# FriedFeid/Video-Depth-Anything

Measured on AMD Instinct MI355X. Metric: depth frames/sec at 32x518x518, ViT-L fp16, 1/2/4/8 MI355X, higher is better.
Workload: dtype fp16; 1 GPU; VideoDepthAnything.forward vitl 1x32x3x518x518 per GPU; encoder=vitl, frames_per_clip=32, H=518, W=518, clips_per_gpu=1, parallelism=clip-parallel dp1, ranks=1, depth_gather_to_rank0=False, hip_graph=False, clips_in_flight=2

## Files before the change

include/vda_tune.h:

```cpp
#ifndef VDA_TUNE_H
#define VDA_TUNE_H
#include <stdint.h>
#ifdef __cplusplus
extern "C" {
#endif

int vda_debug_force_tile(int32_t cfg);
int vda_debug_gemm_sched(int32_t persist_blocks);
int vda_debug_strip_split(int32_t nsplit);
int vda_debug_hconv(int32_t mode);
int vda_debug_dconv(int32_t mode);
int vda_debug_attn(int32_t temporal_direct);

#ifdef __cplusplus
}
#endif
#endif
```

video-depth-anything_amd/_lib.py:

```python
from __future__ import annotations

import ctypes
import os
from ctypes import c_float, c_int32, c_int64, c_void_p, POINTER

_HERE = os.path.dirname(os.path.abspath(__file__))
LIB_PATH = os.environ.get("VDA_LIB_OVERRIDE") or os.path.join(_HERE, "libvda.so")
TORCH_LIB_PATH = os.path.join(_HERE, "libvda_torch.so")
if os.environ.get("VDA_LIB_OVERRIDE"):
    _ov = os.path.join(os.path.dirname(os.path.abspath(os.environ["VDA_LIB_OVERRIDE"])), "libvda_torch.so")
    if os.path.exists(_ov):
        TORCH_LIB_PATH = _ov

EXPORTED = (
    "vda_version", "vda_epilogue_size", "vda_last_error", "vda_gemm", "vda_gemm_check", "vda_conv2d", "vda_conv2d_workspace",
    "vda_layernorm",
    "vda_conv2d_res2_upsample_ok", "vda_conv2d_bias9_ok",
    "vda_subpixel_conv", "vda_subpixel_conv_workspace", "vda_subpixel_conv_check",
    "vda_row_stats", "vda_groupnorm", "vda_groupnorm_workspace",
    "vda_groupnorm_linear", "vda_groupnorm_linear_workspace", "vda_groupnorm_linear_fused",
    "vda_spatial_attention", "vda_temporal_attention", "vda_upsample_bilinear", "vda_patch_im2col",
    "vda_depth_head", "vda_depth_head_workspace", "vda_preprocess_frames", "vda_depth_resize",
    "vda_scale_shift", "vda_scale_shift_workspace", "vda_depth_align",
    "vda_depth_eval_workspace", "vda_depth_eval_fit", "vda_depth_eval_metrics",
    "vda_depth_range_workspace", "vda_depth_range", "vda_depth_colorize_bytes", "vda_depth_colorize",
    "vda_tile_size", "vda_depth_absdiff_range_workspace", "vda_depth_absdiff_range", "vda_panel_compose_bytes",
    "vda_panel_compose",
    "vda_yuv_to_rgb", "vda_preprocess_yuv_workspace", "vda_preprocess_yuv",
    "vda_resample_taps", "vda_resample_tables", "vda_yuv_downscale_ok", "vda_yuv_downscale_workspace",
    "vda_yuv_downscale",
    "vda_gemm_f32", "vda_conv2d_f32", "vda_layernorm_f32", "vda_groupnorm_f32", "vda_spatial_attention_f32",
    "vda_temporal_attention_f32", "vda_upsample_bilinear_f32", "vda_patch_im2col_f32", "vda_depth_head_f32",
)
TUNE_EXPORTED = ("vda_debug_force_tile", "vda_debug_gemm_sched", "vda_debug_strip_split", "vda_debug_hconv",
                 "vda_debug_dconv", "vda_debug_attn")
TUNE_LIB_PATH = os.path.join(os.path.dirname(_HERE), "build", "tune", "libvda.so")

ACT_NONE, ACT_GELU, ACT_GEGLU, ACT_RELU, ACT_SWIGLU = 0, 1, 2, 3, 4
STORE_ROWS, STORE_PIXEL_SHUFFLE = 0, 1
VIS_INDEX, VIS_HWC, VIS_PLANAR444, VIS_PLANAR420 = 0, 1, 2, 3
TILE_RGB, TILE_DEPTH, TILE_ERROR, TILE_XT = 0, 1, 2, 3
YUV_420, YUV_422, YUV_444, YUV_MONO = 0, 1, 2, 3


class VDAUnavailable(RuntimeError):
    pass


class VDAError(RuntimeError):
    pass


class Epilogue(ctypes.Structure):
    _fields_ = [
        ("bias", c_void_p), ("rowbias", c_void_p), ("rdiv", c_int32), ("rmod", c_int32),
        ("gamma", c_void_p), ("res", c_void_p), ("ldres", c_int64), ("res2", c_void_p),
        ("ldres2", c_int64), ("act", c_int32), ("store", c_int32), ("ps_k", c_int32),
        ("ps_cout", c_int32), ("ps_hin", c_int32), ("ps_win", c_int32),
        ("ln_stats", c_void_p), ("ln_colsum", c_void_p), ("ln_parts", c_int32), ("ln_eps", c_float),
        ("stats_out", c_void_p), ("res2_h", c_int32), ("res2_w", c_int32), ("sched", c_void_p),
        ("drop_period", c_int32), ("bias9", c_void_p),
    ]


class Tile(ctypes.Structure):
    _fields_ = [
        ("kind", c_int32), ("row", c_int32), ("col", c_int32), ("offset", c_int32), ("frames", c_int32),
        ("lut", c_int32), ("a", c_void_p), ("b", c_void_p), ("valid", c_void_p), ("range", c_void_p),
    ]


_lib = None
_load_error = None


def _declare(lib):
    P, I, L, F = c_void_p, c_int32, c_int64, c_float
    EP = POINTER(Epilogue)
    sig = {
        "vda_version": ([], ctypes.c_char_p),
        "vda_epilogue_size": ([], L),
        "vda_last_error": ([], ctypes.c_char_p),
        "vda_gemm": ([P, L, P, P, L, I, I, I, EP, P], I),
        "vda_gemm_check": ([L, L, I, I, I, EP], I),
        "vda_conv2d": ([P, P, P, I, I, I, I, I, I, I, I, I, I, I, EP, P, L, P], I),
        "vda_conv2d_workspace": ([I, I, I, I, I, I, I, I], L),
        "vda_conv2d_res2_upsample_ok": ([I, I, I, I, I, I, I, I], I),
        "vda_conv2d_bias9_ok": ([I, I, I, I, I, I, I], I),
        "vda_subpixel_conv": ([P, P, P, P, I, I, I, I, I, I, P, L, P], I),
        "vda_subpixel_conv_workspace": ([I, I, I, I, I], L),
        "vda_subpixel_conv_check": ([I, I, I, I, I, I], I),
        "vda_layernorm": ([P, L, P, P, P, I, I, F, I, P], I),
        "vda_row_stats": ([P, L, P, I, I, F, P], I),
        "vda_groupnorm": ([P, P, P, P, I, I, I, I, F, P, P], I),
        "vda_groupnorm_workspace": ([I, I, I, I], L),
        "vda_groupnorm_linear": ([P, P, P, I, I, I, I, F, P, P, P, I, P, P, L, P], I),
        "vda_groupnorm_linear_workspace": ([I, I, I, I, I], L),
        "vda_groupnorm_linear_fused": ([I, I, I], I),
        "vda_spatial_attention": ([P, P, I, I, I, I, F, P], I),
        "vda_temporal_attention": ([P, P, I, I, I, I, I, F, F, P], I),
        "vda_upsample_bilinear": ([P, P, I, I, I, I, I, I, P], I),
        "vda_patch_im2col": ([P, P, I, I, I, I, P], I),
        "vda_depth_head": ([P, P, P, P, P, P, P, I, I, I, I, I, I, P], I),
        "vda_depth_head_workspace": ([I, I, I, I, I, I], L),
        "vda_preprocess_frames": ([P, P, I, I, I, I, I, POINTER(F), POINTER(F), P], I),
        "vda_depth_resize": ([P, P, I, I, I, I, I, P], I),
        "vda_scale_shift_workspace": ([L], L),
        "vda_scale_shift": ([P, P, P, L, P, P, P, L, P], I),
        "vda_depth_align": ([P, I, I, I, I, I, P, I, P, POINTER(F), POINTER(F), P, P], I),
        "vda_depth_eval_workspace": ([I, L], L),
        "vda_depth_eval_fit": ([P, P, P, I, L, I, P, P, P, L, P], I),
        "vda_depth_eval_metrics": ([P, P, P, I, L, P, I, F, P, P, P, P, L, P], I),
        "vda_depth_range_workspace": ([L], L),
        "vda_depth_range": ([P, L, P, P, L, P], I),
        "vda_depth_colorize_bytes": ([I, I, I, I], L),
        "vda_depth_colorize": ([P, I, I, I, P, P, I, P, P], I),
        "vda_tile_size": ([], L),
        "vda_depth_absdiff_range_workspace": ([L], L),
        "vda_depth_absdiff_range": ([P, P, P, L, P, P, L, P], I),
        "vda_panel_compose_bytes": ([I, I, I, I, I, I], L),
        "vda_panel_compose": ([POINTER(Tile), I, I, I, I, I, I, I, I, I, P, P, I, P, P], I),
        "vda_yuv_to_rgb": ([P, I, I, I, L, I, P, P], I),
        "vda_preprocess_yuv_workspace": ([I, I, I, I, I], L),
        "vda_preprocess_yuv": ([P, I, I, I, L, I, P, I, I, POINTER(F), POINTER(F), P, L, P], I),
        "vda_resample_taps": ([I, I], I),
        "vda_resample_tables": ([I, I, P, P], I),
        "vda_yuv_downscale_ok": ([I, I, I, I], I),
        "vda_yuv_downscale_workspace": ([I, I, I, I, I], L),
        "vda_yuv_downscale": ([P, I, I, I, L, I, P, P, P, P, P, I, I, P, L, P], I),
        "vda_gemm_f32": ([P, L, P, P, L, I, I, I, EP, P], I),
        "vda_conv2d_f32": ([P, P, P, I, I, I, I, I, I, I, I, I, EP, P], I),
        "vda_layernorm_f32": ([P, L, P, P, P, I, I, F, I, P], I),
        "vda_groupnorm_f32": ([P, P, P, P, I, I, I, I, F, P], I),
        "vda_spatial_attention_f32": ([P, P, I, I, I, I, F, P], I),
        "vda_temporal_attention_f32": ([P, P, I, I, I, I, I, F, F, P], I),
        "vda_upsample_bilinear_f32": ([P, P, I, I, I, I, I, I, P], I),
        "vda_patch_im2col_f32": ([P, P, I, I, I, I, P], I),
        "vda_depth_head_f32": ([P, P, P, P, P, P, P, P, I, I, I, I, I, I, P], I),
        "vda_debug_force_tile": ([I], I),
        "vda_debug_gemm_sched": ([I], I),
        "vda_debug_strip_split": ([I], I),
        "vda_debug_hconv": ([I], I),
        "vda_debug_dconv": ([I], I),
        "vda_debug_attn": ([I], I),
    }
    for name, (args, res) in sig.items():
        if name.startswith("vda_debug_") and not hasattr(lib, name):
            continue
        fn = getattr(lib, name)
        fn.argtypes = args
        fn.restype = res


def lib():
    global _lib, _load_error
    if _lib is not None:
        return _lib
    if _load_error is not None:
        raise VDAUnavailable(_load_error)
    if not os.path.exists(LIB_PATH):
        _load_error = f"libvda.so not found at {LIB_PATH}; run `make` (or __graft_entry__.build())"
        raise VDAUnavailable(_load_error)
    try:
        l = ctypes.CDLL(LIB_PATH)
        _declare(l)
        if l.vda_epilogue_size() != ctypes.sizeof(Epilogue):
            raise OSError(f"vda_epilogue is {l.vda_epilogue_size()} bytes in the library, {ctypes.sizeof(Epilogue)} "
                          f"in _lib.Epilogue: rebuild libvda.so or update the mirror")
        if l.vda_tile_size() != ctypes.sizeof(Tile):
            raise OSError(f"vda_tile is {l.vda_tile_size()} bytes in the library, {ctypes.sizeof(Tile)} in _lib.Tile: "
                          f"rebuild libvda.so or update the mirror")
    except OSError as e:
        _load_error = f"failed to load {LIB_PATH}: {e}"
        raise VDAUnavailable(_load_error) from e
    _lib = l
    return _lib


_torch_ops = None


def torch_ops():
    global _torch_ops
    if _torch_ops is not None:
        return _torch_ops
    lib()
    if not os.path.exists(TORCH_LIB_PATH):
        raise VDAUnavailable(f"libvda_torch.so not found at {TORCH_LIB_PATH}; run `make` (or __graft_entry__.build())")
    import torch
    try:
        torch.ops.load_library(TORCH_LIB_PATH)
    except OSError as e:
        raise VDAUnavailable(f"failed to load {TORCH_LIB_PATH}: {e}") from e
    _torch_ops = torch.ops.vda
    return _torch_ops


def check(rc: int, what: str):
    if rc != 0:
        msg = lib().vda_last_error().decode(errors="replace")
        raise VDAError(f"{what} failed (rc={rc}): {msg}")
```

video-depth-anything_amd/csrc/vda_conv2d.hip:

```cpp
#include "vda_internal.h"

static bool conv_takes_strip(int BT, int H, int W, int Cin, int Cout, int ks, int stride, int pad, int up_h) {
  if (up_h > 0 || ks != 3 || stride != 1 || pad != 1 || !vda_conv_strip_serves(W, Cin, Cout)) return false;
  const long strip_tiles = (long)BT * ((H * W + 255) / 256);
  return g_force_tile == -3 || (g_force_tile == -1 && (Cin >= 512 || strip_tiles * 2 <= vda_cu_count()));
}

static long conv_im2col_bytes(int BT, int H, int W, int Cin, int ks, int stride, int pad) {
  const long Ho = (H + 2L * pad - ks) / stride + 1, Wo = (W + 2L * pad - ks) / stride + 1;
  return (long)BT * Ho * Wo * ks * ks * Cin * 2;
}
static bool conv_takes_im2col(int BT, int H, int W, int Cin, int Cout, int ks, int stride, int pad, int up_h) {
  if (up_h > 0 || ks != 3 || stride != 2 || Cout % 256 != 0 || g_force_tile != -1) return false;
  const long Ho = (H + 2L * pad - ks) / stride + 1, Wo = (W + 2L * pad - ks) / stride + 1;
  return Ho > 0 && Wo > 0 && vda_gemm_phased256_serves((long)BT * Ho * Wo, Cout, 9L * Cin, 9L * Cin);
}

static bool conv_takes_hconv(int BT, int H, int W, int Cin, int Cout, int ks, int stride, int pad) {
  return ks == 3 && stride == 1 && pad == 1 && g_force_tile == -1 && vda_conv_hconv_serves(BT, H, W, Cin, Cout);
}

extern "C" int64_t vda_conv2d_workspace(int32_t BT, int32_t H, int32_t W, int32_t Cin, int32_t Cout, int32_t ks,
                                        int32_t stride, int32_t pad) {
  if (BT <= 0 || H <= 0 || W <= 0 || Cin <= 0 || Cout <= 0) return 0;
  if (conv_takes_hconv(BT, H, W, Cin, Cout, ks, stride, pad)) return 0;
  if (conv_takes_im2col(BT, H, W, Cin, Cout, ks, stride, pad, 0)) return conv_im2col_bytes(BT, H, W, Cin, ks, stride, pad);
  if (!conv_takes_strip(BT, H, W, Cin, Cout, ks, stride, pad, 0)) return 0;
  return vda_conv_strip_ws_bytes(BT, H, W, Cin, Cout);
}

extern "C" int vda_conv2d_res2_upsample_ok(int32_t BT, int32_t H, int32_t W, int32_t Cin, int32_t Cout, int32_t ks,
                                           int32_t stride, int32_t pad) {
  if (BT <= 0 || H <= 0 || W <= 0 || Cin <= 0 || Cout <= 0) return 0;
  return conv_takes_hconv(BT, H, W, Cin, Cout, ks, stride, pad) ? 1 : 0;
}

extern "C" int vda_conv2d_bias9_ok(int32_t BT, int32_t H, int32_t W, int32_t Cin, int32_t Cout, int32_t up_h,
                                   int32_t up_w) {
  if (BT <= 0 || H <= 0 || W <= 0 || Cin <= 0 || Cout <= 0 || up_h <= 0 || up_w <= 0 || g_force_tile >= 0) return 0;
  return vda_conv_halo_fused_serves(BT, H, W, up_h, up_w, Cin, Cout) ? 1 : 0;
}

extern "C" int vda_conv2d(const void* x, const void* w, void* y, int32_t BT, int32_t H, int32_t W,
                          int32_t Cin, int32_t Cout, int32_t ks, int32_t stride, int32_t pad,
                          int32_t pre_relu, int32_t up_h, int32_t up_w, const vda_epilogue* epi,
                          void* ws, int64_t ws_bytes, void* stream) {
  VDA_CHECK_ARG(x && w && y, "null pointer");
  VDA_CHECK_ARG(BT > 0 && H > 0 && W > 0 && Cin > 0 && Cout > 0 && ks > 0 && stride > 0 && pad >= 0,
                "bad conv geometry");
  VDA_CHECK_ARG(Cin % 8 == 0 && Cout % 4 == 0, "Cin % 8 and Cout % 4 required");
  const int Hi = up_h > 0 ? up_h : H, Wi = up_w > 0 ? up_w : W;
  GemmParams p{};
  p.x = (const h16*)x; p.w = (const h16*)w; p.y = (h16*)y;
  p.H = H; p.W = W; p.Cin = Cin; p.ks = ks; p.stride = stride; p.pad = pad; p.pre_relu = pre_relu;
  p.up_h = up_h > 0 ? up_h : 0; p.up_w = up_w > 0 ? up_w : 0;
  p.Ho = (Hi + 2 * pad - ks) / stride + 1;
  p.Wo = (Wi + 2 * pad - ks) / stride + 1;
  VDA_CHECK_ARG(p.Ho > 0 && p.Wo > 0, "empty conv output");
  p.M = BT * p.Ho * p.Wo; p.N = Cout; p.K = ks * ks * Cin;
  p.ldy = Cout; p.ldx = 0;
  p.epi = epi ? *epi : vda_default_epi();
  if (p.epi.rdiv <= 0) p.epi.rdiv = 1;
  if (p.epi.rmod <= 0) p.epi.rmod = 1;
  VDA_CHECK_ARG(p.epi.store == VDA_STORE_ROWS && (p.epi.act == VDA_ACT_NONE || p.epi.act == VDA_ACT_RELU),
                "conv: row store, activation none/relu");
  VDA_CHECK_ARG(!p.epi.stats_out && !p.epi.ln_stats, "conv: no LayerNorm fold / row statistics");
  int rc = vda_check_epi(p.epi, p.M, Cout);
  if (rc) return rc;
  const bool res2_up = p.epi.res2_h > 0 || p.epi.res2_w > 0;
  if (res2_up) {
    VDA_CHECK_ARG(p.epi.res2 && p.epi.res2_h > 0 && p.epi.res2_w > 0 && p.epi.ldres2 == Cout && p.up_h == 0 &&
                      !p.epi.gamma && !p.epi.rowbias && (!p.epi.res || p.epi.ldres == Cout) &&
                      p.epi.res2_h <= p.Ho && p.epi.res2_w <= p.Wo &&
                      (long)p.epi.res2_h * p.epi.res2_w * Cout * 2 < (1L << 31) &&
                      conv_takes_hconv(BT, H, W, Cin, Cout, ks, stride, pad),
                  "upsampled res2 needs the halo conv route (vda_conv2d_res2_upsample_ok), a [BT, h <= Ho, w <= Wo, "
                  "Cout] source, no gamma / rowbias / input upsample");
    return vda_conv_hconv(x, w, y, p.epi.bias, p.epi.act == VDA_ACT_RELU, pre_relu, p.epi.res, p.epi.res2,
                          p.epi.res2_h, p.epi.res2_w, BT, H, W, Cin, Cout, (hipStream_t)stream);
  }
  VDA_CHECK_ARG(!p.epi.bias9 || (!p.epi.bias && (uintptr_t)p.epi.bias9 % 16 == 0 && ks == 3 && stride == 1 && pad == 1 &&
                                 !pre_relu && !p.epi.res && !p.epi.res2 && !p.epi.gamma && !p.epi.rowbias &&
                                 vda_conv2d_bias9_ok(BT, H, W, Cin, Cout, p.up_h, p.up_w)),
                "bias9: the 3x3 conv through a fused resize only (vda_conv2d_bias9_ok), 16-byte aligned, in place "
                "of bias, no residual / gamma / rowbias / pre-ReLU");
  if (p.up_h > 0) {
    if (g_force_tile < 0 && ks == 3 && stride == 1 && pad == 1 && !pre_relu && !p.epi.res && !p.epi.res2 &&
        !p.epi.gamma && !p.epi.rowbias) {
      rc = vda_conv_halo_fused(x, w, y, p.epi.bias, p.epi.act == VDA_ACT_RELU, BT, H, W, p.up_h, p.up_w, Cin, Cout,
                               (hipStream_t)stream, p.epi.bias9);
      if (rc != 1) return rc;
    }
    return vda_launch_conv_reg(p, (hipStream_t)stream);
  }
  if (!p.epi.gamma && !p.epi.rowbias && (!p.epi.res || p.epi.ldres == Cout) && (!p.epi.res2 || p.epi.ldres2 == Cout) &&
      conv_takes_hconv(BT, H, W, Cin, Cout, ks, stride, pad)) {
    rc = vda_conv_hconv(x, w, y, p.epi.bias, p.epi.act == VDA_ACT_RELU, pre_relu, p.epi.res, p.epi.res2, 0, 0, BT, H,
                        W, Cin, Cout, (hipStream_t)stream);
    if (rc != 1) return rc;
  }
  if (conv_takes_strip(BT, H, W, Cin, Cout, ks, stride, pad, 0) && !p.epi.gamma && !p.epi.rowbias &&
      (!p.epi.res || p.epi.ldres == Cout) && (!p.epi.res2 || p.epi.ldres2 == Cout)) {
    rc = vda_conv_strip(x, w, y, p.epi.bias, p.epi.act == VDA_ACT_RELU, pre_relu, p.epi.res, p.epi.res2, BT, H, W,
                        Cin, Cout, ws, ws ? ws_bytes : 0, (hipStream_t)stream);
    if (rc != 1) return rc;
  }
  if (g_force_tile < 0 && ks == 3 && stride == 1 && pad == 1 && !pre_relu && !p.epi.res && !p.epi.res2 &&
      !p.epi.gamma && !p.epi.rowbias && (long)H * W >= 128L * 128L) {
    rc = vda_conv_halo(x, w, y, p.epi.bias, p.epi.act == VDA_ACT_RELU, BT, H, W, Cin, Cout, (hipStream_t)stream);
    if (rc != 1) return rc;
  }
  if (conv_takes_im2col(BT, H, W, Cin, Cout, ks, stride, pad, 0) && !pre_relu && ws &&
      ws_bytes >= conv_im2col_bytes(BT, H, W, Cin, ks, stride, pad) && (uintptr_t)ws % 16 == 0 &&
      (uintptr_t)x % 16 == 0) {
    rc = vda_conv_im2col(x, ws, BT, H, W, Cin, p.Ho, p.Wo, ks, stride, pad, (hipStream_t)stream);
    if (rc) return rc;
    p.x = (const h16*)ws;
    p.ldx = p.K;
    return vda_launch_gemm(p, (hipStream_t)stream);
  }
  return vda_launch_conv_gemm(p, (hipStream_t)stream);
}
```

video-depth-anything_amd/csrc/vda_internal.h:

```cpp
#pragma once
#include "vda_common.h"
#include "../../include/vda.h"
static_assert(vda_glu(VDA_ACT_GEGLU) && vda_glu(VDA_ACT_SWIGLU) && !vda_glu(VDA_ACT_GELU) && !vda_glu(VDA_ACT_RELU),
              "vda_glu (vda_common.h) names the gated activation codes of vda.h");

struct GemmParams {
  const h16* x; long ldx;
  const h16* w;
  h16* y; long ldy;
  int M, N, K;
  int H, W, Cin, Ho, Wo, ks, stride, pad, pre_relu, up_h, up_w;
  vda_epilogue epi;
  int sp_bt, sp_phases;
  const float* sp_bias;
};
VDA_KNOB_DECL(int, g_force_tile, -1);
vda_epilogue vda_default_epi();
int vda_check_epi(const vda_epilogue& e, int M, int N);
int vda_launch_gemm(const GemmParams& p, hipStream_t st);
int vda_launch_conv_gemm(const GemmParams& p, hipStream_t st);
bool vda_gemm_phased256_serves(long M, long N, long K, long ldx);
int vda_launch_subpixel_gemm(const GemmParams& p, hipStream_t st);
int vda_launch_conv_reg(const GemmParams& p, hipStream_t st);
int vda_launch_depth_gemm(const GemmParams& p, hipStream_t st);

int vda_conv_halo(const void* x, const void* w, void* y, const float* bias, int relu, int BT, int H, int W, int Cin,
                  int Cout, hipStream_t st);
int vda_conv_halo_fused(const void* x, const void* w, void* y, const float* bias, int relu, int BT, int Hs, int Ws,
                        int H, int W, int Cin, int Cout, hipStream_t st, const float* bias9 = nullptr);
bool vda_conv_halo_fused_serves(int BT, int Hs, int Ws, int H, int W, int Cin, int Cout);

bool vda_depth_conv_serves(int H, int W, int C);
int vda_depth_conv(const void* U, const void* w1, const float* b1, const float* w2, const float* b2, float* depth,
                   int BT, int H, int W, int C, hipStream_t st);
bool vda_depth_conv_fused_serves(int Hs, int Ws, int H, int W, int C);
int vda_depth_conv_fused(const void* x, const void* w1, const float* b1, const float* w2, const float* b2,
                         float* depth, int BT, int Hs, int Ws, int H, int W, int C, hipStream_t st);

bool vda_conv_strip_serves(int W, int Cin, int Cout);
long vda_conv_strip_ws_bytes(int BT, int H, int W, int Cin, int Cout);
int vda_conv_strip(const void* x, const void* w, void* y, const float* bias, int relu_out, int pre_relu,
                   const void* res, const void* res2, int BT, int H, int W, int Cin, int Cout, void* ws,
                   long ws_bytes, hipStream_t st);

bool vda_conv_hconv_serves(int BT, int H, int W, int Cin, int Cout);
int vda_conv_hconv(const void* x, const void* w, void* y, const float* bias, int relu_out, int pre_relu,
                   const void* res, const void* res2, int res2_h, int res2_w, int BT, int H, int W, int Cin, int Cout,
                   hipStream_t st);

int vda_row_partials_launch(const void* y, int64_t ldy, float* out, int32_t rows, int32_t N, hipStream_t st);

int vda_conv_im2col(const void* x, void* a, int BT, int H, int W, int Cin, int Ho, int Wo, int ks, int stride, int pad,
                    hipStream_t st);
```

Baseline: 725.1 frames/s.

## Add source-resolution conv kernel for upsample-then-3x3-conv with Cout 128

Adds a kernel that evaluates a 3x3 conv on a 2x bilinearly upsampled input by running the GEMM on the low-resolution source tile, once per tap, and then applying the separable bilinear weights to the partial results. This cuts the MFMA work to roughly a quarter of convolving the upsampled image and avoids materialising the upsampled halo. The tap outputs are rounded to fp16 in LDS before interpolation, and the path is gated to exact 2x align-corners geometry with Cout=128, Cin<=256 and bias9 present by default. The kernel is tried ahead of the existing halo-fused path.

After: 735.0 frames/s, median of 6. 1.01x the previous value.

```diff
diff --git a/include/vda_tune.h b/include/vda_tune.h
--- a/include/vda_tune.h
+++ b/include/vda_tune.h
@@ -10,6 +10,7 @@
 int vda_debug_strip_split(int32_t nsplit);
 int vda_debug_hconv(int32_t mode);
 int vda_debug_dconv(int32_t mode);
+int vda_debug_oc1_src(int32_t mode);
 int vda_debug_attn(int32_t temporal_direct);
 
 #ifdef __cplusplus
diff --git a/video-depth-anything_amd/_lib.py b/video-depth-anything_amd/_lib.py
--- a/video-depth-anything_amd/_lib.py
+++ b/video-depth-anything_amd/_lib.py
@@ -33,7 +33,7 @@
     "vda_temporal_attention_f32", "vda_upsample_bilinear_f32", "vda_patch_im2col_f32", "vda_depth_head_f32",
 )
 TUNE_EXPORTED = ("vda_debug_force_tile", "vda_debug_gemm_sched", "vda_debug_strip_split", "vda_debug_hconv",
-                 "vda_debug_dconv", "vda_debug_attn")
+                 "vda_debug_dconv", "vda_debug_attn", "vda_debug_oc1_src")
 TUNE_LIB_PATH = os.path.join(os.path.dirname(_HERE), "build", "tune", "libvda.so")
 
 ACT_NONE, ACT_GELU, ACT_GEGLU, ACT_RELU, ACT_SWIGLU = 0, 1, 2, 3, 4
@@ -143,6 +143,7 @@
         "vda_debug_hconv": ([I], I),
         "vda_debug_dconv": ([I], I),
         "vda_debug_attn": ([I], I),
+        "vda_debug_oc1_src": ([I], I),
     }
     for name, (args, res) in sig.items():
         if name.startswith("vda_debug_") and not hasattr(lib, name):
diff --git a/video-depth-anything_amd/csrc/vda_conv2d.hip b/video-depth-anything_amd/csrc/vda_conv2d.hip
--- a/video-depth-anything_amd/csrc/vda_conv2d.hip
+++ b/video-depth-anything_amd/csrc/vda_conv2d.hip
@@ -87,6 +87,9 @@
   if (p.up_h > 0) {
     if (g_force_tile < 0 && ks == 3 && stride == 1 && pad == 1 && !pre_relu && !p.epi.res && !p.epi.res2 &&
         !p.epi.gamma && !p.epi.rowbias) {
+      rc = vda_conv_oc1_src(x, w, y, p.epi.bias, p.epi.act == VDA_ACT_RELU, BT, H, W, p.up_h, p.up_w, Cin, Cout,
+                            (hipStream_t)stream, p.epi.bias9);
+      if (rc != 1) return rc;
       rc = vda_conv_halo_fused(x, w, y, p.epi.bias, p.epi.act == VDA_ACT_RELU, BT, H, W, p.up_h, p.up_w, Cin, Cout,
                                (hipStream_t)stream, p.epi.bias9);
       if (rc != 1) return rc;
diff --git a/video-depth-anything_amd/csrc/vda_internal.h b/video-depth-anything_amd/csrc/vda_internal.h
--- a/video-depth-anything_amd/csrc/vda_internal.h
+++ b/video-depth-anything_amd/csrc/vda_internal.h
@@ -30,6 +30,10 @@
                         int H, int W, int Cin, int Cout, hipStream_t st, const float* bias9 = nullptr);
 bool vda_conv_halo_fused_serves(int BT, int Hs, int Ws, int H, int W, int Cin, int Cout);
 
+bool vda_conv_oc1_src_serves(int BT, int Hs, int Ws, int H, int W, int Cin, int Cout, bool bias9);
+int vda_conv_oc1_src(const void* x, const void* w, void* y, const float* bias, int relu, int BT, int Hs, int Ws, int H,
+                     int W, int Cin, int Cout, hipStream_t st, const float* bias9 = nullptr);
+
 bool vda_depth_conv_serves(int H, int W, int C);
 int vda_depth_conv(const void* U, const void* w1, const float* b1, const float* w2, const float* b2, float* depth,
                    int BT, int H, int W, int C, hipStream_t st);
diff --git a/video-depth-anything_amd/csrc/vda_oc1_src.hip b/video-depth-anything_amd/csrc/vda_oc1_src.hip
--- /dev/null
+++ b/video-depth-anything_amd/csrc/vda_oc1_src.hip
@@ -0,0 +1,348 @@
+#include <cmath>
+#include "vda_internal.h"
+#include "vda_halo.h"
+
+namespace {
+
+__device__ __attribute__((aligned(64))) uint4 g_sz_page[4];
+
+constexpr int ST = 16;
+constexpr int FP = 10;
+constexpr int FPIX = FP * FP;
+constexpr int MROWS = 128;
+constexpr int CMAX = 256;
+constexpr int CS = 64;
+constexpr int CO = 128;
+constexpr int CPX = CS / 8;
+constexpr int ZSTR = 132;
+constexpr int XBUF = MROWS * CMAX;
+constexpr int WBUF = CO * CS;
+constexpr int ZBUF = FPIX * ZSTR;
+constexpr int WPCS = CO * CPX / 64;
+constexpr int WPW = WPCS / 8;
+constexpr int SPS = 2;
+constexpr int WSLOT = SPS * WBUF;
+constexpr int WRING = 2;
+
+#ifndef VDA_OC1S_ABLATE
+#define VDA_OC1S_ABLATE 0
+#endif
+
+typedef unsigned u32x2 __attribute__((ext_vector_type(2)));
+
+__device__ __forceinline__ int w_pos(int n, int cd) { return cd ^ ((n >> 1) & (CPX - 1)); }
+
+__device__ __forceinline__ void slot_weights(int o, int out, int in, float sc, int g, float& a, float& b) {
+  int i0, i1;
+  float w;
+  ac_coord(min(max(o, 0), out - 1), in, sc, i0, i1, w);
+  const float u = 1.f - w;
+  const bool ok = (unsigned)o < (unsigned)out;
+  a = ok ? (i0 == g ? u : 0.f) + (i1 == g ? w : 0.f) : 0.f;
+  b = ok ? (i0 == g + 1 ? u : 0.f) + (i1 == g + 1 ? w : 0.f) : 0.f;
+}
+
+__global__ __launch_bounds__(512) void oc1_src_kernel(const h16* __restrict__ x, const h16* __restrict__ w1,
+                                                      const float* __restrict__ b1, const float* __restrict__ b9,
+                                                      h16* __restrict__ yout, int relu_out, int Hs, int Ws, int C,
+                                                      int tiles_x, int tiles_y, int ntiles) {
+  __shared__ __attribute__((aligned(16))) h16 xbuf[XBUF];
+  __shared__ __attribute__((aligned(16))) h16 wbuf[WRING * WSLOT];
+  __shared__ __attribute__((aligned(16))) h16 zbuf[ZBUF];
+  __shared__ float2 vtab[ST + 2];
+
+  const int tid = threadIdx.x, lane = tid & 63;
+  const int wave = __builtin_amdgcn_readfirstlane(tid >> 6);
+  const int ng = wave & 3, mh = wave >> 2;
+  const int frow = lane & 15, g = lane >> 4;
+  const int H = 2 * Hs, W = 2 * Ws;
+  const int nslab = C / CS;
+  const int K = 9 * C;
+  const int my_tiles = blockIdx.x < ntiles ? (ntiles - 1 - blockIdx.x) / gridDim.x + 1 : 0;
+  if (my_tiles == 0) return;
+  const void* zero = (const void*)g_sz_page;
+  const float usy = ac_scale(Hs, H), usx = ac_scale(Ws, W);
+
+  auto x_rows = [&](int bt, int y0, int x0, const h16* (&xp)[WPW]) {
+    const int by = y0 / 2 - 1, bx = x0 / 2 - 1;
+#pragma unroll
+    for (int j = 0; j < WPW; ++j) {
+      const int s = (wave * WPW + j) * 64 + lane;
+      const int row = s / CPX, cd = w_pos(row, s % CPX);
+      const int r = row / FP, c = row - r * FP;
+      const int gy = by + r, gx = bx + c;
+      const bool ok = row < FPIX && (unsigned)gy < (unsigned)Hs && (unsigned)gx < (unsigned)Ws;
+      xp[j] = ok ? x + (((long)bt * Hs + gy) * Ws + gx) * C + cd * 8 : nullptr;
+    }
+  };
+  auto dma_x_step = [&](const h16* const (&xp)[WPW], int st) {
+#pragma unroll
+    for (int sub = 0; sub < SPS; ++sub) {
+      const int slab = st * SPS + sub;
+#pragma unroll
+      for (int j = 0; j < WPW; ++j)
+        glds16(xp[j] && slab < nslab ? (const void*)(xp[j] + slab * CS) : zero,
+               xbuf + slab * WBUF + (wave * WPW + j) * 512);
+    }
+  };
+  const h16* wrow[WPW];
+#pragma unroll
+  for (int j = 0; j < WPW; ++j) {
+    const int s = (wave * WPW + j) * 64 + lane;
+    const int n = s / CPX, pos = s - n * CPX;
+    wrow[j] = w1 + (long)n * K + w_pos(n, pos) * 8;
+  }
+  const int nstep = (nslab + SPS - 1) / SPS;
+  int pf_tile = 0, pf_tap = 0, pf_step = 0, pf_slot = 0;
+  auto fetch_w = [&]() {
+    if (pf_tile >= my_tiles) return false;
+#if !(VDA_OC1S_ABLATE & 4)
+#pragma unroll
+    for (int sub = 0; sub < SPS; ++sub) {
+      const int slab = pf_step * SPS + sub;
+      const unsigned off = (unsigned)(pf_tap * C + slab * CS);
+#pragma unroll
+      for (int j = 0; j < WPW; ++j)
+        glds16(slab < nslab ? (const void*)(wrow[j] + off) : zero,
+               wbuf + pf_slot * WSLOT + sub * WBUF + (wave * WPW + j) * 512);
+    }
+#endif
+    if (++pf_step == nstep) {
+      pf_step = 0;
+      if (++pf_tap == 9) {
+        pf_tap = 0;
+        ++pf_tile;
+      }
+    }
+    if (++pf_slot == WRING) pf_slot = 0;
+    return true;
+  };
+
+  const int n0r = ng * 32 + frow;
+  unsigned lin_w[2];
+#pragma unroll
+  for (int d = 0; d < 2; ++d)
+    lin_w[d] = (unsigned)(uintptr_t)(VDA_LDS h16*)wbuf + (unsigned)(n0r * CPX + w_pos(n0r, d * 4 + g)) * 16u;
+  unsigned lin_x[2];
+#pragma unroll
+  for (int d = 0; d < 2; ++d)
+    lin_x[d] = (unsigned)(uintptr_t)(VDA_LDS h16*)xbuf +
+               (unsigned)((mh * 64 + frow) * CPX + w_pos(mh * 64 + frow, d * 4 + g)) * 16u;
+  const int xl = tid >> 5, cg = tid & 31;
+
+  const float* bsrc = b9 ? b9 + 4 * CO : b1;
+  const f4 bias_r = bsrc ? *reinterpret_cast<const f4*>(bsrc + cg * 4) : f4{0.f, 0.f, 0.f, 0.f};
+
+  float acc[ST][4];
+#pragma unroll
+  for (int i = 0; i < ST; ++i)
+#pragma unroll
+    for (int c = 0; c < 4; ++c) acc[i][c] = 0.f;
+
+  int bt, y0, x0;
+  halo_tile_of(blockIdx.x, tiles_x, tiles_y, ST, bt, y0, x0);
+  const h16* nxp[WPW];
+  x_rows(bt, y0, x0, nxp);
+  for (int st = 0; st < nstep; ++st) dma_x_step(nxp, st);
+#pragma unroll
+  for (int k = 0; k < WRING - 1; ++k) fetch_w();
+  wait_vmcnt<0>();
+  __builtin_amdgcn_s_barrier();
+
+  int rd_slot = 0;
+  for (int ti = 0; ti < my_tiles; ++ti) {
+    const bool more = ti + 1 < my_tiles;
+    int nbt = 0, ny0 = 0, nx0 = 0;
+    if (more) halo_tile_of(blockIdx.x + (ti + 1) * gridDim.x, tiles_x, tiles_y, ST, nbt, ny0, nx0);
+    if (tid < ST + 2) {
+      float a, b;
+      slot_weights(y0 - 1 + tid, H, Hs, usy, y0 / 2 - 1 + (tid >> 1), a, b);
+      vtab[tid] = make_float2(a, b);
+    }
+    float hA[3], hB[3];
+#pragma unroll
+    for (int tx = 0; tx < 3; ++tx)
+      slot_weights(x0 - 1 + xl + tx, W, Ws, usx, x0 / 2 - 1 + ((xl + tx) >> 1), hA[tx], hB[tx]);
+
+    float hs[FP][4];
+#pragma unroll
+    for (int tap = 0; tap < 9; ++tap) {
+      const int ty = tap / 3, tx = tap % 3;
+      f4 za[2][4];
+#pragma unroll
+      for (int a = 0; a < 2; ++a)
+#pragma unroll
+        for (int i = 0; i < 4; ++i) za[a][i] = f4{0.f, 0.f, 0.f, 0.f};
+      if (tap == 8 && more) x_rows(nbt, ny0, nx0, nxp);
+      for (int st = 0; st < nstep; ++st) {
+        fetch_w();
+        const bool xs = tap == 8 && more && st > 0;
+        if (xs) dma_x_step(nxp, st - 1);
+#if !(VDA_OC1S_ABLATE & 1)
+#pragma unroll
+        for (int d = 0; d < 2 * SPS; ++d) {
+          const int slab = st * SPS + (d >> 1);
+          if (slab < nslab) {
+            const unsigned wa = lin_w[d & 1] + rd_slot * (WSLOT * 2) + (d >> 1) * (WBUF * 2);
+            const unsigned xa = lin_x[d & 1] + slab * (WBUF * 2);
+            u32x4 wf[2], xf[4];
+#pragma unroll
+            for (int a = 0; a < 2; ++a)
+              asm volatile("ds_read_b128 %0, %1 offset:%2" : "=v"(wf[a]) : "v"(wa), "n"(a * 16 * CPX * 16));
+#pragma unroll
+            for (int i = 0; i < 4; ++i)
+              asm volatile("ds_read_b128 %0, %1 offset:%2" : "=v"(xf[i]) : "v"(xa), "n"(i * 16 * CPX * 16));
+            asm volatile("s_waitcnt lgkmcnt(0)"
+                         : "+v"(wf[0]), "+v"(wf[1]), "+v"(xf[0]), "+v"(xf[1]), "+v"(xf[2]), "+v"(xf[3]));
+#pragma unroll
+            for (int a = 0; a < 2; ++a)
+#pragma unroll
+              for (int i = 0; i < 4; ++i)
+                za[a][i] = mfma16(__builtin_bit_cast(h8, wf[a]), __builtin_bit_cast(h8, xf[i]), za[a][i]);
+          }
+        }
+#endif
+        if (xs) wait_vmcnt<SPS * WPW>();
+        else wait_vmcnt<0>();
+        __builtin_amdgcn_s_barrier();
+        rd_slot ^= 1;
+      }
+      if (tap == 8 && more) dma_x_step(nxp, nstep - 1);
+#pragma unroll
+      for (int a = 0; a < 2; ++a)
+#pragma unroll
+        for (int i = 0; i < 4; ++i) {
+          typedef float f2v __attribute__((ext_vector_type(2)));
+          const f4 v = za[a][i];
+          const u32x2 o = {__builtin_bit_cast(unsigned, __builtin_convertvector(f2v{v[0], v[1]}, h2)),
+                           __builtin_bit_cast(unsigned, __builtin_convertvector(f2v{v[2], v[3]}, h2))};
+          const int pix = (mh * 4 + i) * 16 + frow;
+          const h16* dst = zbuf + pix * ZSTR + (ng * 2 + a) * 16 + g * 4;
+          if (pix < FPIX)
+            asm volatile("ds_write_b64 %0, %1" ::"v"((unsigned)(uintptr_t)(VDA_LDS h16*)dst), "v"(o) : "memory");
+        }
+      lgkm0();
+      __builtin_amdgcn_s_barrier();
+#if !(VDA_OC1S_ABLATE & 2)
+      {
+        int t = tid;
+        asm volatile("" : "+v"(t));
+        const h16* zc = zbuf + (((t >> 5) + tx) >> 1) * ZSTR + (t & 31) * 4;
+        const float wa = hA[tx], wb2 = hB[tx];
+#pragma unroll
+        for (int r = 0; r < FP; ++r) {
+          if (r < (ty >> 1) || r > ((ST - 1 + ty) >> 1) + 1) continue;
+          const uint2 p = *reinterpret_cast<const uint2*>(zc + r * FP * ZSTR);
+          const uint2 q = *reinterpret_cast<const uint2*>(zc + r * FP * ZSTR + ZSTR);
+          const float s0 = tx == 0 ? 0.f : hs[r][0], s1 = tx == 0 ? 0.f : hs[r][1];
+          const float s2 = tx == 0 ? 0.f : hs[r][2], s3 = tx == 0 ? 0.f : hs[r][3];
+          hs[r][0] = fma_mix_lo(wb2, q.x, fma_mix_lo(wa, p.x, s0));
+          hs[r][1] = fma_mix_hi(wb2, q.x, fma_mix_hi(wa, p.x, s1));
+          hs[r][2] = fma_mix_lo(wb2, q.y, fma_mix_lo(wa, p.y, s2));
+          hs[r][3] = fma_mix_hi(wb2, q.y, fma_mix_hi(wa, p.y, s3));
+        }
+      }
+      if (tx == 2) {
+#pragma unroll
+        for (int i = 0; i < ST; ++i) {
+          const int k = i + ty;
+          const float2 vw = vtab[k];
+#pragma unroll
+          for (int c = 0; c < 4; ++c)
+            acc[i][c] = __builtin_fmaf(vw.y, hs[(k >> 1) + 1][c], __builtin_fmaf(vw.x, hs[k >> 1][c], acc[i][c]));
+        }
+#pragma unroll
+        for (int i = 0; i < ST; ++i)
+#pragma unroll
+          for (int c = 0; c < 4; ++c) asm volatile("" : "+v"(acc[i][c]));
+      }
+#endif
+    }
+    {
+      const __amdgpu_buffer_rsrc_t ys = __builtin_amdgcn_make_buffer_rsrc(
+          (void*)(yout + (long)bt * H * W * CO), (short)0, (int)((long)H * W * CO * 2), 0x00020000);
+      const bool ring = b9 != nullptr && (y0 == 0 || y0 + ST >= H || x0 == 0 || x0 + ST >= W);
+      const int xg = x0 + xl;
+      const bool odd = (cg & 1) != 0;
+#pragma unroll
+      for (int i = 0; i < ST; i += 2) {
+        u32x2 o[2];
+#pragma unroll
+        for (int e = 0; e < 2; ++e) {
+          const int yg = y0 + i + e;
+          f4 bv = bias_r;
+          if (ring) {
+            const int cls = (yg == 0 ? 0 : yg >= H - 1 ? 2 : 1) * 3 + (xg == 0 ? 0 : xg >= W - 1 ? 2 : 1);
+            bv = *reinterpret_cast<const f4*>(b9 + cls * CO + cg * 4);
+          }
+          h4 h;
+#pragma unroll
+          for (int c = 0; c < 4; ++c) {
+            const float v = acc[i + e][c] + bv[c];
+            h[c] = (h16)(relu_out ? fmaxf(v, 0.f) : v);
+            acc[i + e][c] = 0.f;
+          }
+          o[e] = __builtin_bit_cast(u32x2, h);
+        }
+        const u32x2 snd = odd ? o[0] : o[1];
+        u32x2 rcv;
+        rcv[0] = (unsigned)__builtin_amdgcn_mov_dpp((int)snd[0], 0xB1, 0xF, 0xF, true);
+        rcv[1] = (unsigned)__builtin_amdgcn_mov_dpp((int)snd[1], 0xB1, 0xF, 0xF, true);
+        const u32x4 val = odd ? u32x4{rcv[0], rcv[1], o[1][0], o[1][1]} : u32x4{o[0][0], o[0][1], rcv[0], rcv[1]};
+        const int yg = y0 + i + (odd ? 1 : 0);
+        const unsigned vo = (yg < H && xg < W) ? (unsigned)(((yg * W + xg) * CO + (cg & ~1) * 4) * 2) : 0x80000000u;
+        __builtin_amdgcn_raw_buffer_store_b128(val, ys, vo, 0, 0);
+      }
+    }
+    if (more) {
+      bt = nbt; y0 = ny0; x0 = nx0;
+      wait_vmcnt<ST / 2>();
+      __builtin_amdgcn_s_barrier();
+    }
+  }
+}
+
+bool axis_ok(int n) {
+  const float sc = ac_scale(n, 2 * n);
+  for (int o = 0; o < 2 * n; ++o) {
+    const float f = sc * (float)o;
+    const int i0 = (int)f, i1 = i0 + 1 < n - 1 ? i0 + 1 : n - 1;
+    const float w = std::fmaf(sc, (float)o, -(float)i0);
+    const int ga = ((o + 1) >> 1) - 1;
+    const float kept = (i0 == ga || i0 == ga + 1 ? 1.f - w : 0.f) + (i1 == ga || i1 == ga + 1 ? w : 0.f);
+    if (!(kept > 1.f - 1e-5f)) return false;
+  }
+  return true;
+}
+
+}
+
+VDA_KNOB(int, g_oc1_src, 1);
+
+bool vda_conv_oc1_src_serves(int BT, int Hs, int Ws, int H, int W, int Cin, int Cout, bool bias9) {
+  if (!(g_oc1_src == 2 || (g_oc1_src == 1 && bias9)) || Cout != CO || Cin % CS != 0 || Cin > CMAX || BT < 1 || Hs < 1 || Ws < 1) return false;
+  if (H != 2 * Hs || W != 2 * Ws) return false;
+  if ((long)H * W * Cout * 2 >= (1L << 31)) return false;
+  HaloGrid g;
+  if (!halo_tile_grid(BT, H, W, ST, 1, 0x7fffffffL, g)) return false;
+  return axis_ok(Hs) && axis_ok(Ws);
+}
+
+int vda_conv_oc1_src(const void* x, const void* w, void* y, const float* bias, int relu, int BT, int Hs, int Ws, int H,
+                     int W, int Cin, int Cout, hipStream_t st, const float* bias9) {
+  if (!vda_conv_oc1_src_serves(BT, Hs, Ws, H, W, Cin, Cout, bias9 != nullptr)) return 1;
+  HaloGrid g;
+  halo_tile_grid(BT, H, W, ST, 1, 0x7fffffffL, g);
+  hipLaunchKernelGGL(oc1_src_kernel, dim3(g.grid), dim3(512), 0, st, (const h16*)x, (const h16*)w, bias, bias9,
+                     (h16*)y, relu, Hs, Ws, Cin, g.tiles_x, g.tiles_y, g.ntiles);
+  VDA_LAUNCH_CHECK();
+  return 0;
+}
+
+#ifdef VDA_TUNING
+extern "C" int vda_debug_oc1_src(int32_t mode) {
+  if (mode < 0 || mode > 2) return 1;
+  g_oc1_src = mode;
+  return 0;
+}
+#endif
```
